# svlaskin/bluesky-gym-sasha

Measured on NVIDIA B200. Metric: env_steps_per_sec, higher is better.
Workload: dtype f32 (lat/lon f64)

## Files before the change

bluesky_gym_sasha_b200/csrc/env_kernels.cuh:

```cuda
#pragma once
#include <cuda_runtime.h>
#include <stdint.h>

#include "bsg_internal.h"
#include "bsg_math.cuh"
#include "cd_pair.cuh"
#include "rng.cuh"

namespace bsg {

#ifndef BSG_ENV_THREADS
#define BSG_ENV_THREADS 128
#endif
constexpr int kEnvThreads = BSG_ENV_THREADS;
constexpr int kEnvBlocksPerSm = 896 / BSG_ENV_THREADS;
constexpr uint32_t kFlAlive = 1u, kFlLnav = 2u, kFlLastWp = 4u, kFlTgt = 8u , kFlWpShift = 8u;
enum { kModeStep = 0, kModeReset = 1, kModeTraf = 2 };

enum { PH_NA = 0, PH_TO = 1, PH_IC = 2, PH_CL = 3, PH_CR = 4, PH_DE = 5, PH_AP = 6, PH_LD = 7, PH_GD = 8 };

struct EnvParams {
    int env_type, E, n_int, cd_enabled, autoreset, max_steps, hdg_random, n_sub, fms_rel_freq, mode;
    int obs_dim, act_dim, info_dim;
    int fc_slot;
// ... 297 lines not shown
    }
}

template <bool WIND, bool EXT = false>
__device__ __forceinline__ void ac_kinematics(Ac& a, const EnvParams& P, const Targets& T, const float ext_trk = 0.0f,
                                              const float ext_vs = 0.0f) {
    const float dt = P.simdt;
    const bsg_perf& pf = P.perf;
    float selvs_eff = fabsf(a.selvs) > 0.1f ? a.selvs : kVsDef;
    float p_vs = fabsf(selvs_eff);
    float p_hdg = mod360(a.aptrk);
    if (EXT) { p_vs = fabsf(ext_vs); p_hdg = mod360(ext_trk); }
    float wn = 0.0f, we = 0.0f;
    if (WIND) {
        wind_at(P, a.lat, a.lon, a.alt, wn, we);
        const float vw = sqrtf(fmaf(wn, wn, we * we));
        const float drift = a.aptrk * kDeg2Rad - atan2f(we, wn);
        const float steer = asinf(fminf(1.0f, fmaxf(-1.0f, vw * sinf(drift) / fmaxf(0.001f, a.tas))));
        p_hdg = mod360(a.aptrk + kRad2Deg * steer);
        if (!(a.alt > 50.0f * kFt)) { wn = 0.0f; we = 0.0f; }
    }
    const float amax = T.amax, allow_tas = T.allow_tas, allow_h = T.allow_h;
    float vs_max_acc = (1.0f - a.ax * T.inv_amax) * pf.vsmax;
    float allow_vs = p_vs;
    if (p_vs > 0.0f && p_vs > pf.vsmax) allow_vs = vs_max_acc;
    if (p_vs < 0.0f && p_vs < pf.vsmin) allow_vs = vs_max_acc;
    if (T.ph == PH_GD && a.tas < pf.vminto) allow_vs = 0.0f;
    float dspd = allow_tas - a.tas;
    bool need_ax = fabsf(dspd) > fabsf(dt * amax);
    a.ax = need_ax ? copysignf(amax, dspd) : 0.0f;
    a.tas = need_ax ? a.tas + a.ax * dt : allow_tas;
    float turnrate = (kRad2Deg * (kG0 * kTanBankDef)) * rcp_approx(fmaxf(a.tas, 0.01f));
    float delhdg = degto180(p_hdg - a.hdg);
    bool swhdgsel = fabsf(delhdg) > fabsf(dt * turnrate);
    a.hdg = mod360(swhdgsel ? a.hdg + copysignf(dt * turnrate, delhdg) : p_hdg);
    float delta_alt = allow_h - a.alt;
    bool swaltsel = fabsf(delta_alt) > 1.05f * fmaxf(fabsf(dt * allow_vs), fabsf(dt * a.vs));
    float target_vs = swaltsel ? copysignf(fabsf(allow_vs), delta_alt) : 0.0f;
    float delta_vs = target_vs - a.vs;
    bool need_az = fabsf(delta_vs) > kAzMax;
    a.vs = need_az ? a.vs + copysignf(kAzMax, delta_vs) * dt : target_vs;
    if (!isfinite(a.vs)) a.vs = 0.0f;
    float sh, ch;
    __sincosf((a.hdg - 180.0f) * kDeg2Rad, &sh, &ch);
    a.gsn = -a.tas * ch; a.gse = -a.tas * sh;
    if (WIND) { a.gsn += wn; a.gse += we; }
    a.alt = swaltsel ? a.alt + a.vs * dt : allow_h;
    a.lat += (double)(kRad2Deg * (dt * a.gsn * (1.0f / kRearth)));
    a.coslat = __cosf((float)a.lat * kDeg2Rad);
    a.lon += (double)(kRad2Deg * (dt * a.gse * rcp_approx(a.coslat) * (1.0f / kRearth)));
}

enum { HX = 0, HY = 1, HCH = 2, HSH = 3, HU = 4, HV = 5, kHotFields = 6 };
constexpr int kQueuePerThread = 16;
#ifndef BSG_HOT_UNROLL
#define BSG_HOT_UNROLL 1
#endif
constexpr int kHotUnroll = BSG_HOT_UNROLL;
#ifndef BSG_CD_REUSE
#define BSG_CD_REUSE 1
#endif
constexpr float kCdVelTol = 0.15f;
constexpr float kCdAbsEps = 1.0f;

constexpr int kSmallPairs = 8 * 7 / 2;
__device__ __forceinline__ void build_pair_table(uint16_t* s_pairs) {
    for (int p = threadIdx.x; p < kSmallPairs; p += blockDim.x) {
        int j = (int)((1.0f + sqrtf(1.0f + 8.0f * (float)p)) * 0.5f);
        while (j * (j - 1) / 2 > p) --j;
        while ((j + 1) * j / 2 <= p) ++j;
        int i = p - j * (j - 1) / 2;
        s_pairs[p] = (uint16_t)((i << 8) | j);
    }
}

__device__ __forceinline__ u64 abs2(u64 v) { return v & 0x7fffffff7fffffffULL; }
__device__ __forceinline__ u64 neg2(u64 v) { return v ^ 0x8000000080000000ULL; }

template <int G>
struct __align__(16) GroupSmem {
    float4 rec[2 * G];
    float hot[(G > 8) ? 2 * G * kHotFields : 4];
    uint16_t queue[(G > 8) ? G * kQueuePerThread : 8];
    int tmax[G];
    int cnt, nb, np, pad;
};

#ifdef BSG_SUBSTEP_CLOCKS
__device__ long long g_clk[16];
#define BSG_CLK(k) do { if (clk_on) g_clk[k] = clock64(); } while (0)
#else
#define BSG_CLK(k) do { } while (0)
#endif
template <int G, bool TOL>
__device__ __forceinline__ void group_cd(GroupSmem<G>& S, const int lane_g, Ac& a, bool alive, int nac, const EnvParams& P, float horizon,
                                         const uint16_t* s_pairs, int& nconf_env, int& nlos_env, const bool emit, const int e,
                                         const bool lane_moved, const double lat_ref, const double lon_ref) {
    const int lane = threadIdx.x & 31;
    const int wbase = lane - lane_g;
#ifdef BSG_SUBSTEP_CLOCKS
    const bool clk_on = e == 0 && lane_g == 0 && horizon == 4.0f * P.simdt;
#endif
    BSG_CLK(0);
    const float ch = sqrt_approx(fmaf(0.5f, a.coslat, 0.5f));
    const float sh = __int_as_float((__float_as_int(sqrt_approx(fmaxf(fmaf(-0.5f, a.coslat, 0.5f), 0.0f))) & 0x7fffffff) |
                                    (__double2hiint(a.lat) & 0x80000000));
    const float x = (kRearth * kDeg2Rad) * (float)(a.lon - lon_ref), y = (kRearth * kDeg2Rad) * (float)(a.lat - lat_ref);
    S.rec[2 * lane_g] = make_float4(x, y, ch, sh);
    S.rec[2 * lane_g + 1] = make_float4(a.gse, a.gsn, a.alt, a.vs);
    S.tmax[lane_g] = 0;
    if (emit && lane_g == 0) S.np = 0;
    unsigned confmask = 0u;
    int counts = 0;
    bool found = true;
    auto exact_pair = [&](int i, int j) {
        CdSym r = cd_pair_sym(S.rec[2 * i], S.rec[2 * i + 1], S.rec[2 * j], S.rec[2 * j + 1], P.R2, P.hpz, P.dtlook);
        counts += (r.conf_ij ? 1 : 0) + (r.conf_ji ? 1 : 0) + (r.los ? (2 << 16) : 0);
        confmask |= (r.conf_ij ? 1u << (wbase + i) : 0u) | (r.conf_ji ? 1u << (wbase + j) : 0u);
        if (r.conf_ij | r.conf_ji) {
            const int tb = __float_as_int(fmaxf(r.tcpa, 0.0f));
            if (r.conf_ij) atomicMax(&S.tmax[i], tb);
            if (r.conf_ji) atomicMax(&S.tmax[j], tb);
        }
        if (emit && (r.conf_ij | r.conf_ji | r.los)) {
            const int k = atomicAdd(&S.np, 1);
            if (k < P.cd_pair_cap) {
                const long long o = (long long)e * P.cd_pair_cap + k;
                P.cd_pairs[o] = (uint32_t)i | ((uint32_t)j << 8) | (r.conf_ij ? (uint32_t)BSG_PAIR_CONF_IJ : 0u) |
                                (r.conf_ji ? (uint32_t)BSG_PAIR_CONF_JI : 0u) | (r.los ? (uint32_t)BSG_PAIR_LOS : 0u);
                if (P.cd_attr) {
                    float* q = P.cd_attr + o * BSG_PAIR_ATTR_COUNT;
                    q[BSG_PAIR_ATTR_QDR] = mod360(kRad2Deg * atan2f(r.dx, r.dy));
                    q[BSG_PAIR_ATTR_DIST] = sqrtf(r.dist2);
                    q[BSG_PAIR_ATTR_DCPA] = sqrtf(r.dcpa2);
                    q[BSG_PAIR_ATTR_TCPA] = r.tcpa;
                    q[BSG_PAIR_ATTR_TINCONF_IJ] = r.tin_ij;
                    q[BSG_PAIR_ATTR_TINCONF_JI] = r.tin_ji;
                }
            }
        }
    };
    if (G <= 8) {
        __syncwarp(group_mask<G>());
        const int npairs = nac * (nac - 1) / 2;
        for (int p = lane_g; p < npairs; p += G) {
            const unsigned ij = s_pairs[p];
            exact_pair((int)(ij >> 8), (int)(ij & 0xffu));
        }
    } else {
    const unsigned gm = group_mask<G>();
    const int m = nac - 1, r = lane_g - 1;
    const bool ring = lane_g >= 1 && lane_g < nac;
    const int kmax = m >> 1;
    float* hot = S.hot;
    uint16_t* queue = S.queue;
    const float Rh = P.rpz * 1.0002f, Lh = P.dtlook * 1.0002f;
    int nb = S.nb;
    bool moved;
    if (TOL) moved = ring && (fabsf(a.gse - hot[HU * 2 * G + (lane_g - 1)]) + fabsf(a.gsn - hot[HV * 2 * G + (lane_g - 1)]) > kCdVelTol);
    else moved = ring && lane_moved;
    const bool eval_b = !BSG_CD_REUSE || P.cd_enabled == 2 || nb < 0 || __any_sync(gm, moved);
    u64 KAP = 0, RR = 0, D0 = 0, DW = 0, LH = 0;
    if (eval_b) {
        if (ring) {
            float* w = hot + r;
            w[HX * 2 * G] = -x; w[HY * 2 * G] = y;  w[HCH * 2 * G] = ch;
            w[HSH * 2 * G] = sh; w[HU * 2 * G] = a.gse; w[HV * 2 * G] = a.gsn;
            w += m;
            w[HX * 2 * G] = -x; w[HY * 2 * G] = y;  w[HCH * 2 * G] = ch;
            w[HSH * 2 * G] = sh; w[HU * 2 * G] = a.gse; w[HV * 2 * G] = a.gsn;
        }
        if (lane_g == 0) S.cnt = 0;
        float kap = 0.0f, d0 = 0.0f, dw = 0.0f;
        if (BSG_CD_REUSE && P.cd_enabled != 2 && horizon > 0.0f) {
            const bool in = lane_g < nac;
            const float spd = in ? sqrtf(fmaf(a.gse, a.gse, a.gsn * a.gsn)) : 0.0f;
            const float cl = fmaxf(a.coslat, 0.0175f);
            const float tl = in ? sqrt_approx(fmaxf(fmaf(-cl, cl, 1.0f), 0.0f)) * rcp_approx(cl) * 1.0001f : 0.0f;
            const float vmax = __uint_as_float(__reduce_max_sync(gm, __float_as_uint(spd))) + kCdVelTol;
            const float tmax = __uint_as_float(__reduce_max_sync(gm, __float_as_uint(tl)));
            kap = 1.5f * horizon * vmax * tmax * (1.0f / kRearth);
            d0 = (4.0f * vmax + 1.0f) * horizon;
            dw = TOL ? 2.0f * kCdVelTol : 0.0f;
        }
        KAP = pk2(kap, kap); RR = pk2(fmaf(kap, d0, Rh), fmaf(kap, d0, Rh)); D0 = pk2(d0, d0); DW = pk2(dw, dw);
        const float lh = P.cd_enabled != 2 ? Lh + horizon * 1.0002f : Lh;
        LH = pk2(lh, lh);
    }
    __syncwarp(gm);
    BSG_CLK(1);
    if (eval_b) {
        unsigned cand = 0u;
        {
            const u64 pX = pk2(x, x), nY = pk2(-y, -y), CH = pk2(ch, ch), nSH = pk2(-sh, -sh);
            const u64 nU = pk2(-a.gse, -a.gse), nV = pk2(-a.gsn, -a.gsn);
            const u64 EPS = pk2(kCdAbsEps, kCdAbsEps);
            const float* q = hot + r + 1;
#pragma unroll kHotUnroll
            for (int kk = 0; kk < kmax; kk += 2, q += 2) {
                const u64 nX = pk2(q[HX * 2 * G], q[HX * 2 * G + 1]);
                const u64 Y = pk2(q[HY * 2 * G], q[HY * 2 * G + 1]);
                const u64 CHc = pk2(q[HCH * 2 * G], q[HCH * 2 * G + 1]);
                const u64 SHc = pk2(q[HSH * 2 * G], q[HSH * 2 * G + 1]);
                const u64 U = pk2(q[HU * 2 * G], q[HU * 2 * G + 1]);
                const u64 V = pk2(q[HV * 2 * G], q[HV * 2 * G + 1]);
                const u64 dy = add2(Y, nY);
                const u64 cav = fma2(SHc, nSH, mul2(CHc, CH));
                const u64 ndxl = add2(nX, pX);
                const u64 ndx = mul2(ndxl, cav);
                const u64 du = add2(U, nU), dv = add2(V, nV);
                const u64 dv2 = fma2(du, du, mul2(dv, dv));
                const u64 crs = fma2(ndx, dv, mul2(dy, du));
                const u64 dot = fma2(neg2(du), ndx, mul2(dv, dy));
                float w0, w1;
                up2(dv2, w0, w1);
                const u64 W = add2(pk2(sqrt_approx(w0), sqrt_approx(w1)), DW);
                const u64 l1 = add2(abs2(ndxl), abs2(dy));
                const u64 rm = fma2(KAP, l1, RR);
                const u64 t0 = fma2(W, rm, fma2(add2(l1, D0), DW, EPS));
                const u64 reach = fma2(W, LH, rm);
                float c0, c1, d0, d1, a0, a1, s0, s1, f0, f1;
                up2(abs2(crs), c0, c1);
                up2(dot, d0, d1);
                up2(t0, a0, a1);
                up2(fma2(ndx, ndx, mul2(dy, dy)), s0, s1);
                up2(mul2(reach, reach), f0, f1);
                cand |= (((c0 < a0 && d0 < a0 && s0 < f0) ? 1u : 0u) | ((c1 < a1 && d1 < a1 && s1 < f1) ? 2u : 0u)) << kk;
            }
            unsigned valid = (1u << kmax) - 1u;
            if (!(m & 1) && r >= kmax) valid >>= 1;
            cand = ring ? (cand & valid) : 0u;
        }
        if (__any_sync(gm, cand != 0u)) {
            const int cnt = __popc(cand);
            int pos = 0;
            if (cnt) pos = atomicAdd(&S.cnt, cnt);
            uint16_t* qp = queue + pos;
#pragma unroll 1
            for (unsigned c = cand; c; c &= c - 1u) {
                int rj = r + __ffs(c);
                rj = rj >= m ? rj - m : rj;
                *qp++ = (uint16_t)((lane_g << 8) | (rj + 1));
            }
            __syncwarp(gm);
            nb = S.cnt;
        } else {
            nb = 0;
        }
        if (lane_g == 0) S.nb = nb;
    }
    BSG_CLK(2);
    int ncand;
    {
        const float4 A0 = S.rec[0], B0 = S.rec[1];
        const float cav = fmaf(-A0.w, sh, A0.z * ch);
        const float dx = (x - A0.x) * cav, dy = y - A0.y;
        const float du = a.gse - B0.x, dv = a.gsn - B0.y;
        const float dv2 = fmaf(du, du, dv * dv);
        const float crs = fmaf(dx, dv, -dy * du);
        const float dot = fmaf(du, dx, dv * dy);
        const float w = sqrt_approx(dv2);
        const float t0 = fmaf(w, Rh, kCdAbsEps), reach = fmaf(w, Lh, Rh);
        const bool pass = ring && fabsf(crs) < t0 && dot < t0 && fmaf(dx, dx, dy * dy) < reach * reach;
        const unsigned bm = (G >= 32) ? __ballot_sync(gm, pass) : ((__ballot_sync(gm, pass) >> wbase) & ((1u << (G & 31)) - 1u));
        if (pass) queue[nb + __popc(bm & ((1u << lane_g) - 1u))] = (uint16_t)lane_g;
        ncand = nb + __popc(bm);
        __syncwarp(gm);
    }
    BSG_CLK(3);
    for (int p = lane_g; p < ncand; p += G) {
        const unsigned en = queue[p];
        exact_pair((int)(en >> 8), (int)(en & 0xffu));
    }
    found = ncand > 0;
#ifdef BSG_SUBSTEP_CLOCKS
    if (clk_on) g_clk[8] = ncand;
#endif
    BSG_CLK(4);
    }
    if (found) {
        confmask = __reduce_or_sync(group_mask<G>(), confmask);
        counts = (int)__reduce_add_sync(group_mask<G>(), (unsigned)counts);
    }
    a.inconf = alive && ((confmask >> lane) & 1u);
    a.tcpamax = __int_as_float(S.tmax[lane_g]);
    nconf_env = counts & 0xffff;
    nlos_env = counts >> 16;
    __syncwarp(group_mask<G>());
    BSG_CLK(5);
}

}
```

bluesky_gym_sasha_b200/csrc/env_step.cu:

```cuda
#ifdef BSG_SUBSTEP_CLOCKS
#include <cstdio>
#endif
#include "env_kernels.cuh"

namespace bsg {

struct StepOut { float reward; int terminated; int truncated; };

template <int G>
__device__ __forceinline__ int nearest_rank(float dist, bool cand, int K) {
    const unsigned lane_g = threadIdx.x & (G - 1);
    unsigned long long key = cand ? (((unsigned long long)__float_as_uint(dist)) << 32) | lane_g : ~0ULL;
    int rank = -1;
    for (int r = 0; r < K; ++r) {
        unsigned long long m = group_min_u64<G>(key);
        if (m == key && key != ~0ULL) { rank = r; key = ~0ULL; }
    }
    return rank;
}

__device__ double g_tas150_tab[2001];

template <int G>
__device__ inline void descent_reset(Ac& a, EnvS& s, const EnvParams& P, long long e, int slot) {
// ... 754 lines not shown
                                          bool with_reward) {
    if (ENV == BSG_ENV_DESCENT) return descent_obs_reward<G>(a, s, P, obs, slot, with_reward);
    if (ENV == BSG_ENV_HORIZONTAL_CR) return horizontal_obs_reward<G>(a, s, P, obs, slot, with_reward);
    if (ENV == BSG_ENV_SECTOR_CR) return sector_obs_reward<G>(a, s, P, obs, slot, e, with_reward);
    if (ENV == BSG_ENV_PLAN_WAYPOINT) return planwp_obs_reward<G>(a, s, P, obs, slot, e, with_reward);
    if (ENV == BSG_ENV_VERTICAL_CR) return vertical_obs_reward<G>(a, s, P, obs, slot, with_reward);
    if (ENV == BSG_ENV_STATIC_OBSTACLE) return static_obs_reward<G>(a, s, P, obs, slot, e, with_reward);
    return merge_obs_reward<G>(a, s, P, obs, slot, with_reward);
}
template <int ENV>
__device__ __forceinline__ void do_info(const EnvS& s, const EnvParams& P, const int e) {
    float info[6];
    if (ENV == BSG_ENV_DESCENT) descent_info(s, info);
    else if (ENV == BSG_ENV_MERGE) merge_info(s, info);
    else if (ENV == BSG_ENV_PLAN_WAYPOINT) {
        info[0] = s.total_reward; info[1] = (float)__popc((unsigned)s.wpt_reach); info[2] = 0.0f; info[3] = 0.0f;
    } else if (ENV == BSG_ENV_VERTICAL_CR) {
        info[0] = s.total_reward; info[1] = (float)s.intrusions; info[2] = s.final_alt; info[3] = 0.0f;
    } else if (ENV == BSG_ENV_STATIC_OBSTACLE) {
        info[0] = s.total_reward; info[1] = (float)s.wpt_reach; info[2] = (float)s.intrusions;
        info[3] = s.drift_sum / (float)s.drift_n;
    } else drift_info(s, info);
    info[4] = (float)s.nconf; info[5] = (float)s.nlos;
#pragma unroll
    for (int k = 0; k < 6; ++k) P.info[(long long)k * P.E + e] = info[k];
}

#ifndef BSG_FAST_STEADY
#define BSG_FAST_STEADY 1
#endif
#ifndef BSG_PIN_SLOT
#define BSG_PIN_SLOT 0
#endif
#ifndef BSG_PIN_GROUP
#define BSG_PIN_GROUP 1
#endif
#ifndef BSG_TARGET_CACHE
#define BSG_TARGET_CACHE 1
#endif
#ifdef BSG_PHASE_TIMING
#define BSG_STAMP(k) do { asm volatile("mov.u64 %0, %%globaltimer;" : "=l"(stamps[k]) :: "memory"); } while (0)
#else
#define BSG_STAMP(k) do { } while (0)
#endif

template <int ENV, int G, bool WIND>
__global__ void __launch_bounds__(kEnvThreads, kEnvBlocksPerSm) env_kernel(const EnvParams P) {
    __shared__ GroupSmem<(G > 1) ? G : 2> s_grp[(G > 1) ? kEnvThreads / G : 1];
    __shared__ uint16_t s_pairs[(G > 1 && G <= 8) ? kSmallPairs : 1];
    if (G > 1 && G <= 8 && P.cd_enabled && P.mode != kModeReset) {
        build_pair_table(s_pairs);
        __syncthreads();
    }
    __shared__ double s_scratch[(ENV == BSG_ENV_SECTOR_CR) ? (kEnvThreads / 32) * kSectorScratch
                                : (ENV == BSG_ENV_STATIC_OBSTACLE) ? (kEnvThreads / G) * kStaticScratch : 1];
    const int tid = threadIdx.x;
    const int gt = blockIdx.x * kEnvThreads + tid;
    if (gt == 0 && P.mode == kModeStep && P.final_count) {
        P.final_count[P.fc_slot ^ 1] = 0;
        P.final_count[2] = P.fc_slot;
    }
    const int e = gt / G;
    int slot_ = gt % G;
#if BSG_PIN_SLOT
    asm volatile("" : "+r"(slot_));
#endif
    const int slot = slot_;
    if (e >= P.E) return;
    double* scratch = (ENV == BSG_ENV_SECTOR_CR) ? &s_scratch[(threadIdx.x / 32) * kSectorScratch]
                    : (ENV == BSG_ENV_STATIC_OBSTACLE) ? &s_scratch[(threadIdx.x / G) * kStaticScratch] : s_scratch;
    int grp = (G > 1) ? tid / G : 0;
#if BSG_PIN_GROUP
    asm volatile("" : "+r"(grp));
#endif
    auto& S = s_grp[grp];

#ifdef BSG_PHASE_TIMING
    unsigned long long stamps[8] = {0, 0, 0, 0, 0, 0, 0, 0};
#endif
    BSG_STAMP(0);
    Ac a;
    ac_load(a, P, gt);
    float act[2] = {0.0f, 0.0f};
    if (P.mode == kModeStep) {
        act[0] = P.actions[(long long)e * P.act_dim];
        if (ENV == BSG_ENV_SECTOR_CR || ENV == BSG_ENV_MERGE || ENV == BSG_ENV_STATIC_OBSTACLE) act[1] = P.actions[(long long)e * P.act_dim + 1];
    }
    EnvS s;
    env_load_pre(s, P, e);
    if (slot == 0) {
        asm volatile("prefetch.global.L2 [%0];" ::"l"(P.ef64 + (long long)e * BSG_F64_COUNT));
        asm volatile("prefetch.global.L2 [%0];" ::"l"(P.ef32 + (long long)e * BSG_F32_COUNT));
    }
    if (ENV == BSG_ENV_SECTOR_CR && slot < 4) asm volatile("prefetch.global.L2 [%0];" ::"l"(P.poly + (long long)e * (2 * kSectorMaxV) + 16 * slot));
    float* obs = P.obs + (long long)e * P.obs_dim;

    bool resetting;
    if (P.mode == kModeReset) {
        resetting = P.reset_mask ? (P.reset_mask[e] != 0) : true;
        if (!resetting) return;
    } else {
        resetting = (P.mode == kModeStep) && (P.autoreset == BSG_AUTORESET_NEXT_STEP) && (s.needs_reset != 0);
    }

    if (!resetting) {
        ac_finish_load(a, P);
        const bool alive = (a.flags & kFlAlive) != 0;
        bool tgt_cached = (BSG_TARGET_CACHE && P.mode == kModeStep && (a.flags & kFlTgt) != 0) || !alive;
        if (P.mode == kModeStep) {
            const float o_selspd = a.selspd, o_selalt = a.selalt;
            if (ENV == BSG_ENV_DESCENT || ENV == BSG_ENV_VERTICAL_CR) descent_action<G>(a, P, act, slot);
            if (ENV == BSG_ENV_PLAN_WAYPOINT) horizontal_action<G>(a, P, act, slot);
            if (ENV == BSG_ENV_STATIC_OBSTACLE) static_action<G>(a, P, act, slot);
            if (ENV == BSG_ENV_HORIZONTAL_CR) horizontal_action<G>(a, P, act, slot);
            if (ENV == BSG_ENV_SECTOR_CR) sector_action<G>(a, P, act, slot);
            if (ENV == BSG_ENV_MERGE) merge_action<G>(a, P, act, slot);
            tgt_cached = tgt_cached && a.selspd == o_selspd && a.selalt == o_selalt;
            if (WIND && ENV != BSG_ENV_DESCENT && ENV != BSG_ENV_VERTICAL_CR && slot == 0 && a.alt > 50.0f * kFt) {
                float wn, we, sh, ch;
                wind_at(P, a.lat, a.lon, a.alt, wn, we);
                sincosf(a.aptrk * kDeg2Rad, &sh, &ch);
                a.aptrk = mod360(kRad2Deg * atan2f(fmaf(a.tas, sh, we), fmaf(a.tas, ch, wn)));
            }
        }
        int nconf = s.nconf, nlos = s.nlos;
        if (G > 8 && P.cd_enabled) {
            if (slot == 0) S.nb = -1;
            __syncwarp(group_mask<G>());
        }
        BSG_STAMP(1);
        constexpr bool kNeedAtmos = ENV == BSG_ENV_SECTOR_CR || ENV == BSG_ENV_MERGE || ENV == BSG_ENV_STATIC_OBSTACLE;
        Targets T;
        compute_targets<kNeedAtmos>(a, P, T, tgt_cached);
        BSG_STAMP(2);
        bool fixed = false;
        bool moved = false;
#pragma unroll 1
        for (int k = 0; k < P.n_sub; ++k) {
            s.simk += 1;
            const bool fms_ready = ENV == BSG_ENV_MERGE && (s.simk % P.fms_rel_freq) == 0;
            if (alive) {
                if (a.alt != T.k_alt || a.vs != T.k_vs) compute_targets<true>(a, P, T, false);
                ac_autopilot<ENV>(a, P, fms_ready);
            }
            if constexpr (G > 1) if (P.cd_enabled) {
                const bool emit = P.cd_pairs != nullptr && (k == P.n_sub - 1 || ENV == BSG_ENV_STATIC_OBSTACLE);
                const double lat_ref = ENV == BSG_ENV_MERGE ? P.fix_lat : (ENV == BSG_ENV_SECTOR_CR ? kSectorLat0 : 52.0);
                const double lon_ref = ENV == BSG_ENV_MERGE ? P.fix_lon : (ENV == BSG_ENV_SECTOR_CR ? kSectorLon0 : 4.0);
                group_cd<G, ENV == BSG_ENV_MERGE || WIND>(S, slot, a, alive, s.num_ac, P, (float)(P.n_sub - 1 - k) * P.simdt, s_pairs, nconf,
                                                          nlos, emit, e, moved, lat_ref, lon_ref);
                if (emit && slot == 0) P.ei32[(long long)e * BSG_I32_COUNT + BSG_I32_NPAIRS] = S.np;
            }
#ifdef BSG_SUBSTEP_CLOCKS
            if (e == 0 && slot == 0 && k == P.n_sub - 5) g_clk[6] = clock64();
#endif
            if (BSG_FAST_STEADY && !WIND && ENV != BSG_ENV_MERGE && group_all<G>(fixed || !alive)) {
                moved = false;
                if (alive) {
                    a.lat += (double)(kRad2Deg * (P.simdt * a.gsn * (1.0f / kRearth)));
                    a.coslat = __cosf((float)a.lat * kDeg2Rad);
                    a.lon += (double)(kRad2Deg * (P.simdt * a.gse * rcp_approx(a.coslat) * (1.0f / kRearth)));
                }
            } else if (alive) {
                const float o_tas = a.tas, o_hdg = a.hdg, o_vs = a.vs, o_alt = a.alt, o_ax = a.ax, o_gsn = a.gsn, o_gse = a.gse;
                ac_kinematics<WIND>(a, P, T);
                moved = a.gsn != o_gsn || a.gse != o_gse;
                fixed = !moved && a.tas == o_tas && a.hdg == o_hdg && a.vs == o_vs && a.alt == o_alt && a.ax == o_ax;
            }
#ifdef BSG_SUBSTEP_CLOCKS
            if (e == 0 && slot == 0 && k == P.n_sub - 5) {
                g_clk[7] = clock64();
                printf("substep clocks [cycles]: record+sync %lld | (B) %lld | (A) filter %lld | exact (%lld cand) %lld | merge+readback %lld | to kin %lld | kinematics %lld | whole %lld\n",
                       g_clk[1] - g_clk[0], g_clk[2] - g_clk[1], g_clk[3] - g_clk[2], g_clk[8], g_clk[4] - g_clk[3], g_clk[5] - g_clk[4],
                       g_clk[6] - g_clk[5], g_clk[7] - g_clk[6], g_clk[7] - g_clk[0]);
            }
#endif
            if (ENV == BSG_ENV_STATIC_OBSTACLE && P.mode == kModeStep) {
                if (k == 0) env_load_post(s, P, e);
                if (static_substep_check<G>(a, s, P, e, slot)) break;
            }
#ifdef BSG_PHASE_TIMING
            if (k == 0) BSG_STAMP(3);
#endif
        }
        BSG_STAMP(4);
        if ((kNeedAtmos || P.mode == kModeTraf) && alive && P.n_sub > 0) {
            a.cas = tas2cas(a.tas, T.at);
        }
        a.tgt = T.allow_tas;
        a.flags = (BSG_TARGET_CACHE && alive && T.k_alt == a.alt && T.k_vs == a.vs) ? (a.flags | kFlTgt) : (a.flags & ~kFlTgt);
        s.nconf = nconf; s.nlos = nlos;
        if (P.mode == kModeTraf) {
            ac_store(a, P, gt);
            if (slot == 0) env_store_pre(s, P, e);
            return;
        }
        if (ENV != BSG_ENV_STATIC_OBSTACLE) env_load_post(s, P, e);
    }

#pragma unroll 1
    for (int pass = 0; pass < 2; ++pass) {
        const bool fresh = resetting;
        if (resetting) do_reset<ENV, G>(a, s, P, e, slot, scratch);
        StepOut o = do_obs<ENV, G>(a, s, P, obs, slot, e, !fresh);
        if (P.wind_obs && slot == 0) {
            float wn = 0.0f, we = 0.0f, sh, ch;
            if (WIND) wind_at(P, a.lat, a.lon, a.alt, wn, we);
            sincosf(a.hdg * kDeg2Rad, &sh, &ch);
            obs[P.obs_dim - 2] = (wn * ch + we * sh) * (1.0f / 50.0f);
            obs[P.obs_dim - 1] = (-wn * sh + we * ch) * (1.0f / 50.0f);
        }
#ifdef BSG_PHASE_TIMING
        if (pass == 0) BSG_STAMP(5);
#endif
        if (pass == 1) break;
        if (fresh) {
            if (slot == 0) { P.reward[e] = 0.0f; P.term[e] = 0; P.trunc[e] = 0; do_info<ENV>(s, P, e); }
            break;
        }
        s.step += 1;
        if (P.max_steps > 0 && s.step >= P.max_steps) o.truncated = 1;
        if (slot == 0) {
            P.reward[e] = o.reward; P.term[e] = (uint8_t)o.terminated; P.trunc[e] = (uint8_t)o.truncated;
            do_info<ENV>(s, P, e);
        }
        if (!(o.terminated || o.truncated)) break;
        if (P.autoreset == BSG_AUTORESET_NEXT_STEP) { s.needs_reset = 1; break; }
        if (P.autoreset != BSG_AUTORESET_SAME_STEP) break;
        if (P.final_obs) {
            int k = 0;
            if (slot == 0) { k = atomicAdd(P.final_count + P.fc_slot, 1); P.final_ids[k] = (int32_t)e; }
            k = group_bcast<G>(k, 0);
            __syncwarp(group_mask<G>());
            float* fo = P.final_obs + (long long)k * P.obs_dim;
            for (int i = slot; i < P.obs_dim; i += G) fo[i] = obs[i];
            __syncwarp(group_mask<G>());
        }
// ... 57 lines not shown
```

Baseline: 128.8 million.

## Batch conflict detection across substeps with a ring of snapshot records

For groups larger than 8 lanes, conflict detection is split up. Each substep records a position snapshot into a ring of up to kCdBatch slots, and the exact candidate evaluation is deferred until the ring fills, the filter must be redone, or the last substep arrives. The deferred pass then processes all buffered substeps together in one flat loop over (substep, neighbour) items spread across the lanes. This amortises synchronisation and the per-substep launch of the exact phase and keeps lanes busier. In exchange it adds shared-memory ring storage, reuses the hot staging and sector scratch inside the ring, and makes conflict flags only current at batch boundaries.

```diff
diff --git a/bluesky_gym_sasha_b200/csrc/env_kernels.cuh b/bluesky_gym_sasha_b200/csrc/env_kernels.cuh
--- a/bluesky_gym_sasha_b200/csrc/env_kernels.cuh
+++ b/bluesky_gym_sasha_b200/csrc/env_kernels.cuh
@@ -373,6 +373,11 @@
 }
 
 enum { HX = 0, HY = 1, HCH = 2, HSH = 3, HU = 4, HV = 5, kHotFields = 6 };
+#ifndef BSG_CD_BATCH
+#define BSG_CD_BATCH 4
+#endif
+constexpr int kCdBatch = BSG_CD_BATCH;
+static_assert(kCdBatch >= 3 && kCdBatch <= 16, "BSG_CD_BATCH out of range");
 constexpr int kQueuePerThread = 16;
 #ifndef BSG_HOT_UNROLL
 #define BSG_HOT_UNROLL 1
@@ -400,98 +405,110 @@
 
 template <int G>
 struct __align__(16) GroupSmem {
-    float4 rec[2 * G];
-    float hot[(G > 8) ? 2 * G * kHotFields : 4];
-    uint16_t queue[(G > 8) ? G * kQueuePerThread : 8];
-    int tmax[G];
+    static constexpr bool kBatched = G > 8;
+    static constexpr int kRing = kBatched ? kCdBatch : 1;
+    float4 rec[kRing][2 * G];
+    uint16_t queue[kBatched ? G * kQueuePerThread + kCdBatch * G : 8];
+    int tmax[kRing][G];
+    float2 bvel[kBatched ? G : 1];
     int cnt, nb, np, pad;
 };
 
 #ifdef BSG_SUBSTEP_CLOCKS
-__device__ long long g_clk[16];
-#define BSG_CLK(k) do { if (clk_on) g_clk[k] = clock64(); } while (0)
+#define BSG_CLK(k) do { if (clk_on) { const long long t_ = clock64(); clk_acc[k] += t_ - clk_t; clk_t = t_; } } while (0)
 #else
 #define BSG_CLK(k) do { } while (0)
 #endif
-template <int G, bool TOL>
-__device__ __forceinline__ void group_cd(GroupSmem<G>& S, const int lane_g, Ac& a, bool alive, int nac, const EnvParams& P, float horizon,
-                                         const uint16_t* s_pairs, int& nconf_env, int& nlos_env, const bool emit, const int e,
-                                         const bool lane_moved, const double lat_ref, const double lon_ref) {
+
+__device__ __forceinline__ void cd_emit_pair(const EnvParams& P, int* np, const int e, const int i, const int j, const CdSym& r) {
+    const int k = atomicAdd(np, 1);
+    if (k < P.cd_pair_cap) {
+        const long long o = (long long)e * P.cd_pair_cap + k;
+        P.cd_pairs[o] = (uint32_t)i | ((uint32_t)j << 8) | (r.conf_ij ? (uint32_t)BSG_PAIR_CONF_IJ : 0u) |
+                        (r.conf_ji ? (uint32_t)BSG_PAIR_CONF_JI : 0u) | (r.los ? (uint32_t)BSG_PAIR_LOS : 0u);
+        if (P.cd_attr) {
+            float* q = P.cd_attr + o * BSG_PAIR_ATTR_COUNT;
+            q[BSG_PAIR_ATTR_QDR] = mod360(kRad2Deg * atan2f(r.dx, r.dy));
+            q[BSG_PAIR_ATTR_DIST] = sqrtf(r.dist2);
+            q[BSG_PAIR_ATTR_DCPA] = sqrtf(r.dcpa2);
+            q[BSG_PAIR_ATTR_TCPA] = r.tcpa;
+            q[BSG_PAIR_ATTR_TINCONF_IJ] = r.tin_ij;
+            q[BSG_PAIR_ATTR_TINCONF_JI] = r.tin_ji;
+        }
+    }
+}
+
+template <int G>
+__device__ __forceinline__ void cd_record(GroupSmem<G>& S, const int j, const int lane_g, const Ac& a, const double lat_ref,
+                                          const double lon_ref, float& x, float& y, float& ch, float& sh) {
+    ch = sqrt_approx(fmaf(0.5f, a.coslat, 0.5f));
+    sh = __int_as_float((__float_as_int(sqrt_approx(fmaxf(fmaf(-0.5f, a.coslat, 0.5f), 0.0f))) & 0x7fffffff) |
+                        (__double2hiint(a.lat) & 0x80000000));
+    x = (kRearth * kDeg2Rad) * (float)(a.lon - lon_ref);
+    y = (kRearth * kDeg2Rad) * (float)(a.lat - lat_ref);
+    S.rec[j][2 * lane_g] = make_float4(x, y, ch, sh);
+    S.rec[j][2 * lane_g + 1] = make_float4(a.gse, a.gsn, a.alt, a.vs);
+}
+
+template <int G>
+__device__ __forceinline__ void group_cd_small(GroupSmem<G>& S, const int lane_g, Ac& a, bool alive, int nac, const EnvParams& P,
+                                               const uint16_t* s_pairs, int& nconf_env, int& nlos_env, const bool emit, const int e,
+                                               const double lat_ref, const double lon_ref) {
+    static_assert(G <= 8, "groups of more than 8 lanes detect in batches");
     const int lane = threadIdx.x & 31;
     const int wbase = lane - lane_g;
-#ifdef BSG_SUBSTEP_CLOCKS
-    const bool clk_on = e == 0 && lane_g == 0 && horizon == 4.0f * P.simdt;
-#endif
-    BSG_CLK(0);
-    const float ch = sqrt_approx(fmaf(0.5f, a.coslat, 0.5f));
-    const float sh = __int_as_float((__float_as_int(sqrt_approx(fmaxf(fmaf(-0.5f, a.coslat, 0.5f), 0.0f))) & 0x7fffffff) |
-                                    (__double2hiint(a.lat) & 0x80000000));
-    const float x = (kRearth * kDeg2Rad) * (float)(a.lon - lon_ref), y = (kRearth * kDeg2Rad) * (float)(a.lat - lat_ref);
-    S.rec[2 * lane_g] = make_float4(x, y, ch, sh);
-    S.rec[2 * lane_g + 1] = make_float4(a.gse, a.gsn, a.alt, a.vs);
-    S.tmax[lane_g] = 0;
+    float x, y, ch, sh;
+    cd_record<G>(S, 0, lane_g, a, lat_ref, lon_ref, x, y, ch, sh);
+    S.tmax[0][lane_g] = 0;
     if (emit && lane_g == 0) S.np = 0;
     unsigned confmask = 0u;
     int counts = 0;
-    bool found = true;
-    auto exact_pair = [&](int i, int j) {
-        CdSym r = cd_pair_sym(S.rec[2 * i], S.rec[2 * i + 1], S.rec[2 * j], S.rec[2 * j + 1], P.R2, P.hpz, P.dtlook);
+    __syncwarp(group_mask<G>());
+    const int npairs = nac * (nac - 1) / 2;
+    for (int p = lane_g; p < npairs; p += G) {
+        const unsigned ij = s_pairs[p];
+        const int i = (int)(ij >> 8), j = (int)(ij & 0xffu);
+        const CdSym r = cd_pair_sym(S.rec[0][2 * i], S.rec[0][2 * i + 1], S.rec[0][2 * j], S.rec[0][2 * j + 1], P.R2, P.hpz, P.dtlook);
         counts += (r.conf_ij ? 1 : 0) + (r.conf_ji ? 1 : 0) + (r.los ? (2 << 16) : 0);
         confmask |= (r.conf_ij ? 1u << (wbase + i) : 0u) | (r.conf_ji ? 1u << (wbase + j) : 0u);
         if (r.conf_ij | r.conf_ji) {
             const int tb = __float_as_int(fmaxf(r.tcpa, 0.0f));
-            if (r.conf_ij) atomicMax(&S.tmax[i], tb);
-            if (r.conf_ji) atomicMax(&S.tmax[j], tb);
-        }
-        if (emit && (r.conf_ij | r.conf_ji | r.los)) {
-            const int k = atomicAdd(&S.np, 1);
-            if (k < P.cd_pair_cap) {
-                const long long o = (long long)e * P.cd_pair_cap + k;
-                P.cd_pairs[o] = (uint32_t)i | ((uint32_t)j << 8) | (r.conf_ij ? (uint32_t)BSG_PAIR_CONF_IJ : 0u) |
-                                (r.conf_ji ? (uint32_t)BSG_PAIR_CONF_JI : 0u) | (r.los ? (uint32_t)BSG_PAIR_LOS : 0u);
-                if (P.cd_attr) {
-                    float* q = P.cd_attr + o * BSG_PAIR_ATTR_COUNT;
-                    q[BSG_PAIR_ATTR_QDR] = mod360(kRad2Deg * atan2f(r.dx, r.dy));
-                    q[BSG_PAIR_ATTR_DIST] = sqrtf(r.dist2);
-                    q[BSG_PAIR_ATTR_DCPA] = sqrtf(r.dcpa2);
-                    q[BSG_PAIR_ATTR_TCPA] = r.tcpa;
-                    q[BSG_PAIR_ATTR_TINCONF_IJ] = r.tin_ij;
-                    q[BSG_PAIR_ATTR_TINCONF_JI] = r.tin_ji;
-                }
-            }
-        }
-    };
-    if (G <= 8) {
-        __syncwarp(group_mask<G>());
-        const int npairs = nac * (nac - 1) / 2;
-        for (int p = lane_g; p < npairs; p += G) {
-            const unsigned ij = s_pairs[p];
-            exact_pair((int)(ij >> 8), (int)(ij & 0xffu));
-        }
-    } else {
+            if (r.conf_ij) atomicMax(&S.tmax[0][i], tb);
+            if (r.conf_ji) atomicMax(&S.tmax[0][j], tb);
+        }
+        if (emit && (r.conf_ij | r.conf_ji | r.los)) cd_emit_pair(P, &S.np, e, i, j, r);
+    }
+    confmask = __reduce_or_sync(group_mask<G>(), confmask);
+    counts = (int)__reduce_add_sync(group_mask<G>(), (unsigned)counts);
+    a.inconf = alive && ((confmask >> lane) & 1u);
+    a.tcpamax = __int_as_float(S.tmax[0][lane_g]);
+    nconf_env = counts & 0xffff;
+    nlos_env = counts >> 16;
+    __syncwarp(group_mask<G>());
+}
+
+template <int G, bool TOL>
+__device__ __forceinline__ void cd_filter_b(GroupSmem<G>& S, const int lane_g, const Ac& a, const int nac, const EnvParams& P,
+                                            const float horizon, const float x, const float y, const float ch, const float sh) {
+    static_assert(2 * G * kHotFields * sizeof(float) <= (GroupSmem<G>::kRing - 1) * sizeof(S.rec[0]), "staging > ring slots 1..");
     const unsigned gm = group_mask<G>();
     const int m = nac - 1, r = lane_g - 1;
     const bool ring = lane_g >= 1 && lane_g < nac;
     const int kmax = m >> 1;
-    float* hot = S.hot;
-    uint16_t* queue = S.queue;
+    float* hot = reinterpret_cast<float*>(S.rec[1]);
     const float Rh = P.rpz * 1.0002f, Lh = P.dtlook * 1.0002f;
-    int nb = S.nb;
-    bool moved;
-    if (TOL) moved = ring && (fabsf(a.gse - hot[HU * 2 * G + (lane_g - 1)]) + fabsf(a.gsn - hot[HV * 2 * G + (lane_g - 1)]) > kCdVelTol);
-    else moved = ring && lane_moved;
-    const bool eval_b = !BSG_CD_REUSE || P.cd_enabled == 2 || nb < 0 || __any_sync(gm, moved);
     u64 KAP = 0, RR = 0, D0 = 0, DW = 0, LH = 0;
-    if (eval_b) {
-        if (ring) {
-            float* w = hot + r;
-            w[HX * 2 * G] = -x; w[HY * 2 * G] = y;  w[HCH * 2 * G] = ch;
-            w[HSH * 2 * G] = sh; w[HU * 2 * G] = a.gse; w[HV * 2 * G] = a.gsn;
-            w += m;
-            w[HX * 2 * G] = -x; w[HY * 2 * G] = y;  w[HCH * 2 * G] = ch;
-            w[HSH * 2 * G] = sh; w[HU * 2 * G] = a.gse; w[HV * 2 * G] = a.gsn;
-        }
-        if (lane_g == 0) S.cnt = 0;
+    if (ring) {
+        float* w = hot + r;
+        w[HX * 2 * G] = -x; w[HY * 2 * G] = y;  w[HCH * 2 * G] = ch;
+        w[HSH * 2 * G] = sh; w[HU * 2 * G] = a.gse; w[HV * 2 * G] = a.gsn;
+        w += m;
+        w[HX * 2 * G] = -x; w[HY * 2 * G] = y;  w[HCH * 2 * G] = ch;
+        w[HSH * 2 * G] = sh; w[HU * 2 * G] = a.gse; w[HV * 2 * G] = a.gsn;
+        if (TOL) S.bvel[lane_g] = make_float2(a.gse, a.gsn);
+    }
+    if (lane_g == 0) S.cnt = 0;
+    {
         float kap = 0.0f, d0 = 0.0f, dw = 0.0f;
         if (BSG_CD_REUSE && P.cd_enabled != 2 && horizon > 0.0f) {
             const bool in = lane_g < nac;
@@ -509,105 +526,149 @@
         LH = pk2(lh, lh);
     }
     __syncwarp(gm);
-    BSG_CLK(1);
-    if (eval_b) {
-        unsigned cand = 0u;
-        {
-            const u64 pX = pk2(x, x), nY = pk2(-y, -y), CH = pk2(ch, ch), nSH = pk2(-sh, -sh);
-            const u64 nU = pk2(-a.gse, -a.gse), nV = pk2(-a.gsn, -a.gsn);
-            const u64 EPS = pk2(kCdAbsEps, kCdAbsEps);
-            const float* q = hot + r + 1;
+    unsigned cand = 0u;
+    {
+        const u64 pX = pk2(x, x), nY = pk2(-y, -y), CH = pk2(ch, ch), nSH = pk2(-sh, -sh);
+        const u64 nU = pk2(-a.gse, -a.gse), nV = pk2(-a.gsn, -a.gsn);
+        const u64 EPS = pk2(kCdAbsEps, kCdAbsEps);
+        const float* q = hot + r + 1;
 #pragma unroll kHotUnroll
-            for (int kk = 0; kk < kmax; kk += 2, q += 2) {
-                const u64 nX = pk2(q[HX * 2 * G], q[HX * 2 * G + 1]);
-                const u64 Y = pk2(q[HY * 2 * G], q[HY * 2 * G + 1]);
-                const u64 CHc = pk2(q[HCH * 2 * G], q[HCH * 2 * G + 1]);
-                const u64 SHc = pk2(q[HSH * 2 * G], q[HSH * 2 * G + 1]);
-                const u64 U = pk2(q[HU * 2 * G], q[HU * 2 * G + 1]);
-                const u64 V = pk2(q[HV * 2 * G], q[HV * 2 * G + 1]);
-                const u64 dy = add2(Y, nY);
-                const u64 cav = fma2(SHc, nSH, mul2(CHc, CH));
-                const u64 ndxl = add2(nX, pX);
-                const u64 ndx = mul2(ndxl, cav);
-                const u64 du = add2(U, nU), dv = add2(V, nV);
-                const u64 dv2 = fma2(du, du, mul2(dv, dv));
-                const u64 crs = fma2(ndx, dv, mul2(dy, du));
-                const u64 dot = fma2(neg2(du), ndx, mul2(dv, dy));
-                float w0, w1;
-                up2(dv2, w0, w1);
-                const u64 W = add2(pk2(sqrt_approx(w0), sqrt_approx(w1)), DW);
-                const u64 l1 = add2(abs2(ndxl), abs2(dy));
-                const u64 rm = fma2(KAP, l1, RR);
-                const u64 t0 = fma2(W, rm, fma2(add2(l1, D0), DW, EPS));
-                const u64 reach = fma2(W, LH, rm);
-                float c0, c1, d0, d1, a0, a1, s0, s1, f0, f1;
-                up2(abs2(crs), c0, c1);
-                up2(dot, d0, d1);
-                up2(t0, a0, a1);
-                up2(fma2(ndx, ndx, mul2(dy, dy)), s0, s1);
-                up2(mul2(reach, reach), f0, f1);
-                cand |= (((c0 < a0 && d0 < a0 && s0 < f0) ? 1u : 0u) | ((c1 < a1 && d1 < a1 && s1 < f1) ? 2u : 0u)) << kk;
-            }
-            unsigned valid = (1u << kmax) - 1u;
-            if (!(m & 1) && r >= kmax) valid >>= 1;
-            cand = ring ? (cand & valid) : 0u;
-        }
-        if (__any_sync(gm, cand != 0u)) {
-            const int cnt = __popc(cand);
-            int pos = 0;
-            if (cnt) pos = atomicAdd(&S.cnt, cnt);
-            uint16_t* qp = queue + pos;
+        for (int kk = 0; kk < kmax; kk += 2, q += 2) {
+            const u64 nX = pk2(q[HX * 2 * G], q[HX * 2 * G + 1]);
+            const u64 Y = pk2(q[HY * 2 * G], q[HY * 2 * G + 1]);
+            const u64 CHc = pk2(q[HCH * 2 * G], q[HCH * 2 * G + 1]);
+            const u64 SHc = pk2(q[HSH * 2 * G], q[HSH * 2 * G + 1]);
+            const u64 U = pk2(q[HU * 2 * G], q[HU * 2 * G + 1]);
+            const u64 V = pk2(q[HV * 2 * G], q[HV * 2 * G + 1]);
+            const u64 dy = add2(Y, nY);
+            const u64 cav = fma2(SHc, nSH, mul2(CHc, CH));
+            const u64 ndxl = add2(nX, pX);
+            const u64 ndx = mul2(ndxl, cav);
+            const u64 du = add2(U, nU), dv = add2(V, nV);
+            const u64 dv2 = fma2(du, du, mul2(dv, dv));
+            const u64 crs = fma2(ndx, dv, mul2(dy, du));
+            const u64 dot = fma2(neg2(du), ndx, mul2(dv, dy));
+            float w0, w1;
+            up2(dv2, w0, w1);
+            const u64 W = add2(pk2(sqrt_approx(w0), sqrt_approx(w1)), DW);
+            const u64 l1 = add2(abs2(ndxl), abs2(dy));
+            const u64 rm = fma2(KAP, l1, RR);
+            const u64 t0 = fma2(W, rm, fma2(add2(l1, D0), DW, EPS));
+            const u64 reach = fma2(W, LH, rm);
+            float c0, c1, d0, d1, a0, a1, s0, s1, f0, f1;
+            up2(abs2(crs), c0, c1);
+            up2(dot, d0, d1);
+            up2(t0, a0, a1);
+            up2(fma2(ndx, ndx, mul2(dy, dy)), s0, s1);
+            up2(mul2(reach, reach), f0, f1);
+            cand |= (((c0 < a0 && d0 < a0 && s0 < f0) ? 1u : 0u) | ((c1 < a1 && d1 < a1 && s1 < f1) ? 2u : 0u)) << kk;
+        }
+        unsigned valid = (1u << kmax) - 1u;
+        if (!(m & 1) && r >= kmax) valid >>= 1;
+        cand = ring ? (cand & valid) : 0u;
+    }
+    int nb = 0;
+    if (__any_sync(gm, cand != 0u)) {
+        const int cnt = __popc(cand);
+        int pos = 0;
+        if (cnt) pos = atomicAdd(&S.cnt, cnt);
+        uint16_t* qp = S.queue + pos;
 #pragma unroll 1
-            for (unsigned c = cand; c; c &= c - 1u) {
-                int rj = r + __ffs(c);
-                rj = rj >= m ? rj - m : rj;
-                *qp++ = (uint16_t)((lane_g << 8) | (rj + 1));
-            }
-            __syncwarp(gm);
-            nb = S.cnt;
+        for (unsigned c = cand; c; c &= c - 1u) {
+            int rj = r + __ffs(c);
+            rj = rj >= m ? rj - m : rj;
+            *qp++ = (uint16_t)((lane_g << 8) | (rj + 1));
+        }
+        __syncwarp(gm);
+        nb = S.cnt;
+    }
+    if (lane_g == 0) S.nb = nb;
+}
+
+__device__ __forceinline__ int small_div(const int t, const float r) { return (int)(((float)t + 0.5f) * r); }
+
+template <int G>
+__device__ __forceinline__ void cd_detect_batch(GroupSmem<G>& S, const int lane_g, Ac& a, const bool alive, const int nac,
+                                                const int ns, const EnvParams& P, const bool emit, const int e,
+                                                int& nconf_env, int& nlos_env
+#ifdef BSG_SUBSTEP_CLOCKS
+                                                , long long* clk_acc
+#endif
+                                                ) {
+    const unsigned gm = group_mask<G>();
+    const int wbase = (threadIdx.x & 31) - lane_g;
+#ifdef BSG_SUBSTEP_CLOCKS
+    const bool clk_on = e == 0 && lane_g == 0;
+    long long clk_t = clock64();
+#endif
+#pragma unroll 1
+    for (int s = 0; s < ns; ++s) S.tmax[s][lane_g] = -1;
+    if (emit && lane_g == 0) S.np = 0;
+    __syncwarp(gm);
+    const int nb = S.nb;
+    const float Rh = P.rpz * 1.0002f, Lh = P.dtlook * 1.0002f;
+    const int m = nac - 1, nitems = ns * m;
+    const float rm = rcp_approx((float)m);
+    int na = 0;
+#pragma unroll 1
+    for (int t0 = 0; t0 < nitems; t0 += G) {
+        const int t = t0 + lane_g;
+        bool pass = false;
+        unsigned item = 0u;
+        if (t < nitems) {
+            const int s = small_div(t, rm), j = t - s * m + 1;
+            const float4 A0 = S.rec[s][0], B0 = S.rec[s][1], R = S.rec[s][2 * j], V = S.rec[s][2 * j + 1];
+            const float cav = fmaf(-A0.w, R.w, A0.z * R.z);
+            const float dx = (R.x - A0.x) * cav, dy = R.y - A0.y;
+            const float du = V.x - B0.x, dv = V.y - B0.y;
+            const float dv2 = fmaf(du, du, dv * dv);
+            const float crs = fmaf(dx, dv, -dy * du);
+            const float dot = fmaf(du, dx, dv * dy);
+            const float w = sqrt_approx(dv2);
+            const float tc = fmaf(w, Rh, kCdAbsEps), reach = fmaf(w, Lh, Rh);
+            pass = fabsf(crs) < tc && dot < tc && fmaf(dx, dx, dy * dy) < reach * reach;
+            item = ((unsigned)s << 8) | (unsigned)j;
+        }
+        const unsigned bm = (G >= 32) ? __ballot_sync(gm, pass) : ((__ballot_sync(gm, pass) >> wbase) & ((1u << (G & 31)) - 1u));
+        if (pass) S.queue[nb + na + __popc(bm & ((1u << lane_g) - 1u))] = (uint16_t)item;
+        na += __popc(bm);
+    }
+    __syncwarp(gm);
+    BSG_CLK(3);
+    const int nbs = nb * ns, ncand = nbs + na, sl = ns - 1;
+    const float rnb = rcp_approx((float)nb);
+    int counts = 0;
+#pragma unroll 1
+    for (int t = lane_g; t < ncand; t += G) {
+        int s, i, j;
+        if (t < nbs) {
+            s = small_div(t, rnb);
+            const unsigned en = S.queue[t - s * nb];
+            i = (int)(en >> 8); j = (int)(en & 0xffu);
         } else {
-            nb = 0;
-        }
-        if (lane_g == 0) S.nb = nb;
-    }
-    BSG_CLK(2);
-    int ncand;
-    {
-        const float4 A0 = S.rec[0], B0 = S.rec[1];
-        const float cav = fmaf(-A0.w, sh, A0.z * ch);
-        const float dx = (x - A0.x) * cav, dy = y - A0.y;
-        const float du = a.gse - B0.x, dv = a.gsn - B0.y;
-        const float dv2 = fmaf(du, du, dv * dv);
-        const float crs = fmaf(dx, dv, -dy * du);
-        const float dot = fmaf(du, dx, dv * dy);
-        const float w = sqrt_approx(dv2);
-        const float t0 = fmaf(w, Rh, kCdAbsEps), reach = fmaf(w, Lh, Rh);
-        const bool pass = ring && fabsf(crs) < t0 && dot < t0 && fmaf(dx, dx, dy * dy) < reach * reach;
-        const unsigned bm = (G >= 32) ? __ballot_sync(gm, pass) : ((__ballot_sync(gm, pass) >> wbase) & ((1u << (G & 31)) - 1u));
-        if (pass) queue[nb + __popc(bm & ((1u << lane_g) - 1u))] = (uint16_t)lane_g;
-        ncand = nb + __popc(bm);
-        __syncwarp(gm);
-    }
-    BSG_CLK(3);
-    for (int p = lane_g; p < ncand; p += G) {
-        const unsigned en = queue[p];
-        exact_pair((int)(en >> 8), (int)(en & 0xffu));
-    }
-    found = ncand > 0;
-#ifdef BSG_SUBSTEP_CLOCKS
-    if (clk_on) g_clk[8] = ncand;
-#endif
+            const unsigned en = S.queue[nb + (t - nbs)];
+            s = (int)(en >> 8); i = 0; j = (int)(en & 0xffu);
+        }
+        const CdSym r = cd_pair_sym(S.rec[s][2 * i], S.rec[s][2 * i + 1], S.rec[s][2 * j], S.rec[s][2 * j + 1], P.R2, P.hpz, P.dtlook);
+        if (r.conf_ij | r.conf_ji) {
+            const int tb = __float_as_int(fmaxf(r.tcpa, 0.0f));
+            if (r.conf_ij) atomicMax(&S.tmax[s][i], tb);
+            if (r.conf_ji) atomicMax(&S.tmax[s][j], tb);
+        }
+        if (s == sl) {
+            counts += (r.conf_ij ? 1 : 0) + (r.conf_ji ? 1 : 0) + (r.los ? (2 << 16) : 0);
+            if (emit && (r.conf_ij | r.conf_ji | r.los)) cd_emit_pair(P, &S.np, e, i, j, r);
+        }
+    }
+    counts = (int)__reduce_add_sync(gm, (unsigned)counts);
+    __syncwarp(gm);
     BSG_CLK(4);
-    }
-    if (found) {
-        confmask = __reduce_or_sync(group_mask<G>(), confmask);
-        counts = (int)__reduce_add_sync(group_mask<G>(), (unsigned)counts);
-    }
-    a.inconf = alive && ((confmask >> lane) & 1u);
-    a.tcpamax = __int_as_float(S.tmax[lane_g]);
+    const int tm = S.tmax[sl][lane_g];
+    a.inconf = alive && tm >= 0;
+    a.tcpamax = __int_as_float(max(tm, 0));
     nconf_env = counts & 0xffff;
     nlos_env = counts >> 16;
-    __syncwarp(group_mask<G>());
+    __syncwarp(gm);
     BSG_CLK(5);
 }
 
diff --git a/bluesky_gym_sasha_b200/csrc/env_step.cu b/bluesky_gym_sasha_b200/csrc/env_step.cu
--- a/bluesky_gym_sasha_b200/csrc/env_step.cu
+++ b/bluesky_gym_sasha_b200/csrc/env_step.cu
@@ -830,8 +830,8 @@
         build_pair_table(s_pairs);
         __syncthreads();
     }
-    __shared__ double s_scratch[(ENV == BSG_ENV_SECTOR_CR) ? (kEnvThreads / 32) * kSectorScratch
-                                : (ENV == BSG_ENV_STATIC_OBSTACLE) ? (kEnvThreads / G) * kStaticScratch : 1];
+    static_assert(ENV != BSG_ENV_SECTOR_CR || (G == 32 && sizeof(s_grp[0]) >= kSectorScratch * sizeof(double)), "sector scratch");
+    __shared__ double s_scratch[(ENV == BSG_ENV_STATIC_OBSTACLE) ? (kEnvThreads / G) * kStaticScratch : 1];
     const int tid = threadIdx.x;
     const int gt = blockIdx.x * kEnvThreads + tid;
     if (gt == 0 && P.mode == kModeStep && P.final_count) {
@@ -845,7 +845,7 @@
 #endif
     const int slot = slot_;
     if (e >= P.E) return;
-    double* scratch = (ENV == BSG_ENV_SECTOR_CR) ? &s_scratch[(threadIdx.x / 32) * kSectorScratch]
+    double* scratch = (ENV == BSG_ENV_SECTOR_CR) ? reinterpret_cast<double*>(&s_grp[threadIdx.x / 32])
                     : (ENV == BSG_ENV_STATIC_OBSTACLE) ? &s_scratch[(threadIdx.x / G) * kStaticScratch] : s_scratch;
     int grp = (G > 1) ? tid / G : 0;
 #if BSG_PIN_GROUP
@@ -902,10 +902,6 @@
             }
         }
         int nconf = s.nconf, nlos = s.nlos;
-        if (G > 8 && P.cd_enabled) {
-            if (slot == 0) S.nb = -1;
-            __syncwarp(group_mask<G>());
-        }
         BSG_STAMP(1);
         constexpr bool kNeedAtmos = ENV == BSG_ENV_SECTOR_CR || ENV == BSG_ENV_MERGE || ENV == BSG_ENV_STATIC_OBSTACLE;
         Targets T;
@@ -913,25 +909,38 @@
         BSG_STAMP(2);
         bool fixed = false;
         bool moved = false;
+        const double lat_ref = ENV == BSG_ENV_MERGE ? P.fix_lat : (ENV == BSG_ENV_SECTOR_CR ? kSectorLat0 : 52.0);
+        const double lon_ref = ENV == BSG_ENV_MERGE ? P.fix_lon : (ENV == BSG_ENV_SECTOR_CR ? kSectorLon0 : 4.0);
+        int cdq = 1;
+#ifdef BSG_SUBSTEP_CLOCKS
+        const bool clk_on = e == 0 && slot == 0;
+        long long clk_t = 0, clk_acc[8] = {0, 0, 0, 0, 0, 0, 0, 0};
+        const long long clk_loop = clock64();
+#endif
 #pragma unroll 1
         for (int k = 0; k < P.n_sub; ++k) {
+#ifdef BSG_SUBSTEP_CLOCKS
+            clk_t = clock64();
+#endif
             s.simk += 1;
             const bool fms_ready = ENV == BSG_ENV_MERGE && (s.simk % P.fms_rel_freq) == 0;
             if (alive) {
                 if (a.alt != T.k_alt || a.vs != T.k_vs) compute_targets<true>(a, P, T, false);
                 ac_autopilot<ENV>(a, P, fms_ready);
             }
-            if constexpr (G > 1) if (P.cd_enabled) {
-                const bool emit = P.cd_pairs != nullptr && (k == P.n_sub - 1 || ENV == BSG_ENV_STATIC_OBSTACLE);
-                const double lat_ref = ENV == BSG_ENV_MERGE ? P.fix_lat : (ENV == BSG_ENV_SECTOR_CR ? kSectorLat0 : 52.0);
-                const double lon_ref = ENV == BSG_ENV_MERGE ? P.fix_lon : (ENV == BSG_ENV_SECTOR_CR ? kSectorLon0 : 4.0);
-                group_cd<G, ENV == BSG_ENV_MERGE || WIND>(S, slot, a, alive, s.num_ac, P, (float)(P.n_sub - 1 - k) * P.simdt, s_pairs, nconf,
-                                                          nlos, emit, e, moved, lat_ref, lon_ref);
+            if constexpr (G > 8) if (P.cd_enabled) {
+                float x, y, ch, sh;
+                cd_record<G>(S, cdq >> 1, slot, a, lat_ref, lon_ref, x, y, ch, sh);
+                BSG_CLK(0);
+                if (cdq & 1) cd_filter_b<G, ENV == BSG_ENV_MERGE || WIND>(S, slot, a, s.num_ac, P, (float)(P.n_sub - 1 - k) * P.simdt,
+                                                                           x, y, ch, sh);
+                BSG_CLK(1);
+            }
+            if constexpr (G > 1 && G <= 8) if (P.cd_enabled) {
+                const bool emit = P.cd_pairs != nullptr && k == P.n_sub - 1;
+                group_cd_small<G>(S, slot, a, alive, s.num_ac, P, s_pairs, nconf, nlos, emit, e, lat_ref, lon_ref);
                 if (emit && slot == 0) P.ei32[(long long)e * BSG_I32_COUNT + BSG_I32_NPAIRS] = S.np;
             }
-#ifdef BSG_SUBSTEP_CLOCKS
-            if (e == 0 && slot == 0 && k == P.n_sub - 5) g_clk[6] = clock64();
-#endif
             if (BSG_FAST_STEADY && !WIND && ENV != BSG_ENV_MERGE && group_all<G>(fixed || !alive)) {
                 moved = false;
                 if (alive) {
@@ -945,22 +954,51 @@
                 moved = a.gsn != o_gsn || a.gse != o_gse;
                 fixed = !moved && a.tas == o_tas && a.hdg == o_hdg && a.vs == o_vs && a.alt == o_alt && a.ax == o_ax;
             }
-#ifdef BSG_SUBSTEP_CLOCKS
-            if (e == 0 && slot == 0 && k == P.n_sub - 5) {
-                g_clk[7] = clock64();
-                printf("substep clocks [cycles]: record+sync %lld | (B) %lld | (A) filter %lld | exact (%lld cand) %lld | merge+readback %lld | to kin %lld | kinematics %lld | whole %lld\n",
-                       g_clk[1] - g_clk[0], g_clk[2] - g_clk[1], g_clk[3] - g_clk[2], g_clk[8], g_clk[4] - g_clk[3], g_clk[5] - g_clk[4],
-                       g_clk[6] - g_clk[5], g_clk[7] - g_clk[6], g_clk[7] - g_clk[0]);
-            }
-#endif
+            bool done = false;
             if (ENV == BSG_ENV_STATIC_OBSTACLE && P.mode == kModeStep) {
                 if (k == 0) env_load_post(s, P, e);
-                if (static_substep_check<G>(a, s, P, e, slot)) break;
+                done = static_substep_check<G>(a, s, P, e, slot);
+            }
+            if constexpr (G > 8) if (P.cd_enabled) {
+                const bool ring = slot >= 1 && slot < s.num_ac;
+                bool mv = ring && moved;
+                if (ENV == BSG_ENV_MERGE || WIND) {
+                    const float2 bv = S.bvel[slot];
+                    mv = ring && (fabsf(a.gse - bv.x) + fabsf(a.gsn - bv.y) > kCdVelTol);
+                }
+                const bool refilter = !BSG_CD_REUSE || P.cd_enabled == 2 || __any_sync(group_mask<G>(), mv);
+                BSG_CLK(2);
+                const bool last = done || k == P.n_sub - 1;
+                const int ns = (cdq >> 1) + 1;
+                cdq = (ns << 1) | (refilter ? 1 : 0);
+                if (last || refilter || ns == kCdBatch) {
+                    const bool emit = last && P.cd_pairs != nullptr;
+                    cd_detect_batch<G>(S, slot, a, alive, s.num_ac, ns, P, emit, e, nconf, nlos
+#ifdef BSG_SUBSTEP_CLOCKS
+                                       , clk_acc
+#endif
+                                       );
+                    if (emit && slot == 0) P.ei32[(long long)e * BSG_I32_COUNT + BSG_I32_NPAIRS] = S.np;
+#ifdef BSG_SUBSTEP_CLOCKS
+                    if (clk_on) clk_acc[6] += 1;
+#endif
+#ifdef BSG_PHASE_TIMING
+                    if (k + 1 == ns) BSG_STAMP(3);
+#endif
+                    cdq &= 1;
+                }
             }
 #ifdef BSG_PHASE_TIMING
-            if (k == 0) BSG_STAMP(3);
-#endif
-        }
+            if (k == 0 && (G <= 8 || !P.cd_enabled)) BSG_STAMP(3);
+#endif
+            if (done) break;
+        }
+#ifdef BSG_SUBSTEP_CLOCKS
+        if (clk_on && G > 8 && P.cd_enabled && P.n_sub > 0)
+            printf("substep clocks [cycles, env 0, %d substeps, %lld batches]: record %lld | (B) pass %lld | kinematics + vote %lld | "
+                   "(A) filter %lld | exact %lld | read-back %lld | whole loop %lld\n", P.n_sub, clk_acc[6], clk_acc[0], clk_acc[1], clk_acc[2],
+                   clk_acc[3], clk_acc[4], clk_acc[5], clock64() - clk_loop);
+#endif
         BSG_STAMP(4);
         if ((kNeedAtmos || P.mode == kModeTraf) && alive && P.n_sub > 0) {
             a.cas = tas2cas(a.tas, T.at);
```

New measurement: 126.4 million (median of 6 runs). 0.981x the previous value.
